# zju3dv/LoFTR

Hardware: AMD Instinct MI355X
Metric: image-pairs/sec @640x480 indoor-ds (higher is better)
Workload: dtype f32; 1 GPU; batch=8 640x480 synthetic grayscale pairs per GPU, indoor_ds dual-softmax (BASELINE configs[1]), full LoFTR.forward = ResNet-FPN backbone (HIP implicit-GEMM / patch convolutions incl. the 7x7 stem) + HIP matching path; weights=seeded random init (no checkpoint on the box), conf_matrix_materialised=True, match_type=dual_softmax, global_batch=8, parallelism=dp1 (pairs sharded; RCCL all-gather of match counts)

## Files before the change

loftr_amd/build.py:

```python
import os
import subprocess
import sys
from concurrent.futures import ThreadPoolExecutor

HERE = os.path.dirname(os.path.abspath(__file__))
CSRC = os.path.join(HERE, "csrc")
OBJ_DIR = os.path.join(CSRC, "build")
LIB_PATH = os.path.join(HERE, "libloftr_hip.so")
SOURCES = ["linear.hip", "coarse_plan.hip", "attention.hip", "transformer.hip", "coarse_match.hip", "fine.hip", "misc.hip",
           "sp_convert.hip", "conv.hip", "eval.hip", "input.hip", "comm.hip", "pose.hip", "train.hip", "train_bwd.hip", "encoder_fused.hip", "fine_fused.hip", "head_grads.hip", "encoder_bwd.hip", "fine_bwd.hip", "train_glue.hip", "bank.hip", "pose_gpu.hip", "window_head.hip", "window_head_first.hip", "geometry.hip", "geometry_gpu.hip", "absolute_pose.hip", "absolute_pose_gpu.hip", "atlas.hip", "atlas_gpu.hip", "triangulate.hip", "triangulate_gpu.hip", "model_lookup.hip", "model_lookup_gpu.hip", "bundle.hip", "bundle_gpu.hip", "register.hip", "register_gpu.hip"]
FLAGS = ["--offload-arch=gfx950", "-O3", "-std=c++17", "-fPIC", "-Wall", "-Wno-unused-parameter"]


def _hipcc():
    for c in (os.environ.get("HIPCC"), "/opt/rocm/bin/hipcc", "hipcc"):
        if c and (os.path.isabs(c) and os.path.exists(c) or not os.path.isabs(c)):
            return c
    raise RuntimeError("hipcc not found")


def _deps_mtime():
    paths = [os.path.join(CSRC, f) for f in os.listdir(CSRC) if f.endswith((".h", ".hip"))]
    paths.append(os.path.join(os.path.dirname(HERE), "include", "loftr_hip.h"))
    return max(os.path.getmtime(p) for p in paths)


def build(force=False, verbose=True, extra_flags=(), lib_path=None, obj_dir=None):
    global LIB_PATH, OBJ_DIR
    lib_default, obj_default = LIB_PATH, OBJ_DIR
    if lib_path:
        LIB_PATH, OBJ_DIR, force = lib_path, obj_dir or (OBJ_DIR + "_variant"), True
    try:
        return _build(force, verbose, tuple(extra_flags))
    finally:
        LIB_PATH, OBJ_DIR = lib_default, obj_default


def _build(force, verbose, extra_flags):
    if not force and os.path.exists(LIB_PATH) and os.path.getmtime(LIB_PATH) >= _deps_mtime():
        return LIB_PATH
    os.makedirs(OBJ_DIR, exist_ok=True)
    hipcc = _hipcc()

    def compile_one(src):
        obj = os.path.join(OBJ_DIR, src.replace(".hip", ".o"))
        cmd = [hipcc, *FLAGS, *extra_flags, "-c", os.path.join(CSRC, src), "-o", obj]
        r = subprocess.run(cmd, capture_output=True, text=True)
        if r.returncode != 0:
            raise RuntimeError(f"hipcc failed on {src}:\n{r.stderr}")
        if verbose and r.stderr.strip():
            sys.stderr.write(r.stderr)
        return obj

    with ThreadPoolExecutor(max_workers=min(8, len(SOURCES))) as ex:
        objs = list(ex.map(compile_one, SOURCES))
    vs = os.path.join(OBJ_DIR, "exports.map")
    with open(vs, "w") as fh:
        fh.write("{ global: loftr_*; local: *; };\n")
    r = subprocess.run([hipcc, "--offload-arch=gfx950", "-shared", "-fPIC", f"-Wl,--version-script={vs}", "-o", LIB_PATH, *objs, "-ldl"],
                       capture_output=True, text=True)
    if r.returncode != 0:
        raise RuntimeError(f"link failed:\n{r.stderr}")
    if verbose:
        print(f"built {LIB_PATH} ({os.path.getsize(LIB_PATH) / 1e6:.2f} MB)")
    return LIB_PATH


if __name__ == "__main__":
    if "--variant" in sys.argv:
        i = sys.argv.index("--variant")
        name = sys.argv[i + 1]
        build(extra_flags=[a for a in sys.argv[i + 2:] if a.startswith("-")],
              lib_path=os.path.join(HERE, f"libloftr_hip_{name}.so"), obj_dir=os.path.join(CSRC, "build", f"variant_{name}"))
    else:
        build(force="--force" in sys.argv)
```

loftr_amd/csrc/common.h:

```cpp
#pragma once
#include <hip/hip_runtime.h>
#include <stdint.h>
#include <stddef.h>
#include "../../include/loftr_hip.h"

typedef float f32x16 __attribute__((ext_vector_type(16)));
typedef float f32x4 __attribute__((ext_vector_type(4)));
typedef float f32x2 __attribute__((ext_vector_type(2)));

#define LOFTR_NEG_INF (-1e9f)

#define LOFTR_CHECK_ARG(cond) do { if (!(cond)) return LOFTR_ERR_BAD_ARG; } while (0)
#define LOFTR_CHECK_LAUNCH() do { if (hipGetLastError() != hipSuccess) return LOFTR_ERR_LAUNCH; } while (0)

#ifdef __HIP_DEVICE_COMPILE__
#define LOFTR_NO_PACKED_FP32 __attribute__((target("no-packed-fp32-ops")))
#else
#define LOFTR_NO_PACKED_FP32
#endif

__host__ __device__ static inline int ceil_div(int a, int b) { return (a + b - 1) / b; }
static inline size_t align_up(size_t x, size_t a) { return (x + a - 1) / a * a; }

enum LoftrTimedKernel {
  LOFTR_T_SCORE_STATS = 0,
  LOFTR_T_SCORE_CONF = 1,
  LOFTR_T_PROJ = 2,
  LOFTR_T_LINEAR = 3,
  LOFTR_T_LINEAR_LN = 4,
  LOFTR_T_KV = 5,
  LOFTR_T_ATTN_APPLY = 6,
  LOFTR_T_ATTN_SMALL = 7,
  LOFTR_T_GATHER = 8,
  LOFTR_T_OT_STORE = 9,
  LOFTR_T_CONV = 10,
  LOFTR_T_CONV3 = 11,
  LOFTR_T_CONV3W = 12,
  LOFTR_T_ENCODER_X = 13,
  LOFTR_T_FINE_PAIR = 14,
  LOFTR_T_COUNT = 15
};
enum LoftrDebugKey {
  LOFTR_DBG_ENCODER_SCHEDULE = 0,
  LOFTR_DBG_CONV_PERSIST_CAP,
  LOFTR_DBG_WGRAD_CHUNK,
  LOFTR_DBG_REDUCE_TALL,
  LOFTR_DBG_PCT_GRID,
  LOFTR_DBG_PCT_SKIP,
  LOFTR_DBG_PCT_QUOTA,
  LOFTR_DBG_CONV_DUO,
  LOFTR_DBG_CONV_PATCH,
  LOFTR_DBG_CONV_REM,
  LOFTR_DBG_COUNT
};
int loftr_debug_value(int key);
extern unsigned g_loftr_timing_mask;
extern int g_loftr_range_check;
void loftr_timing_mark(int id, hipStream_t st, bool end);
struct TimedLaunch {
  int id; hipStream_t st; bool on;
  TimedLaunch(int id_, hipStream_t st_) : id(id_), st(st_), on((g_loftr_timing_mask >> id_) & 1u) {
    if (on) loftr_timing_mark(id, st, false);
  }
  ~TimedLaunch() { if (on) loftr_timing_mark(id, st, true); }
};

constexpr int NUM_XCD = 8;
static inline unsigned xcd_grid(int tiles_m, int tiles_n) { return (unsigned)(NUM_XCD * ceil_div(tiles_m, NUM_XCD) * tiles_n); }
__device__ __forceinline__ bool xcd_tile(int tiles_m, int tiles_n, int& tile_m, int& tile_n) {
  const int id = blockIdx.x, xcd = id % NUM_XCD, slot = id / NUM_XCD;
  const int chunk = ceil_div(tiles_m, NUM_XCD);
  tile_n = slot % tiles_n;
  const int local = slot / tiles_n;
  tile_m = xcd * chunk + local;
  return local < chunk && tile_m < tiles_m;
}

struct WsAlloc {
  char* base; size_t cap; size_t off;
  WsAlloc(void* p, size_t bytes) : base((char*)p), cap(bytes), off(0) {}
  template <typename T> T* take(size_t n) {
    off = align_up(off, 256);
    T* r = (T*)(base + off);
    off += n * sizeof(T);
    return r;
  }
  bool ok() const { return off <= cap; }
};

__device__ __forceinline__ float wave_sum(float v) {
#pragma unroll
  for (int o = 32; o >= 1; o >>= 1) v += __shfl_xor(v, o, 64);
  return v;
}
__device__ __forceinline__ float wave_max(float v) {
#pragma unroll
  for (int o = 32; o >= 1; o >>= 1) v = fmaxf(v, __shfl_xor(v, o, 64));
  return v;
}
#define LOFTR_DPP(v_, ctrl_) __int_as_float(__builtin_amdgcn_update_dpp(0, __float_as_int(v_), ctrl_, 0xF, 0xF, true))
#define LOFTR_DPPI(v_, ctrl_) __builtin_amdgcn_update_dpp(0, v_, ctrl_, 0xF, 0xF, true)
__device__ __forceinline__ float half_sum(float v) {
  v += LOFTR_DPP(v, 0xB1);
  v += LOFTR_DPP(v, 0x4E);
  v += LOFTR_DPP(v, 0x141);
  v += LOFTR_DPP(v, 0x140);
  const auto r = __builtin_amdgcn_permlane16_swap(__float_as_int(v), __float_as_int(v), false, false);
  return __int_as_float(r[0]) + __int_as_float(r[1]);
}
__device__ __forceinline__ float half_max(float v) {
  v = fmaxf(v, LOFTR_DPP(v, 0xB1));
  v = fmaxf(v, LOFTR_DPP(v, 0x4E));
  v = fmaxf(v, LOFTR_DPP(v, 0x141));
  v = fmaxf(v, LOFTR_DPP(v, 0x140));
  const auto r = __builtin_amdgcn_permlane16_swap(__float_as_int(v), __float_as_int(v), false, false);
  return fmaxf(__int_as_float(r[0]), __int_as_float(r[1]));
}
__device__ __forceinline__ int half_min_i32(int v) {
  v = min(v, LOFTR_DPPI(v, 0xB1));
  v = min(v, LOFTR_DPPI(v, 0x4E));
  v = min(v, LOFTR_DPPI(v, 0x141));
  v = min(v, LOFTR_DPPI(v, 0x140));
  const auto r = __builtin_amdgcn_permlane16_swap(v, v, false, false);
  return min((int)r[0], (int)r[1]);
}
__device__ __forceinline__ void half_sum16(f32x16& v) {
#pragma unroll
  for (int r = 0; r < 16; ++r) v[r] += LOFTR_DPP(v[r], 0xB1);
#pragma unroll
  for (int r = 0; r < 16; ++r) v[r] += LOFTR_DPP(v[r], 0x4E);
#pragma unroll
  for (int r = 0; r < 16; ++r) v[r] += LOFTR_DPP(v[r], 0x141);
#pragma unroll
  for (int r = 0; r < 16; ++r) v[r] += LOFTR_DPP(v[r], 0x140);
#pragma unroll
  for (int r = 0; r < 16; ++r) {
    const auto q = __builtin_amdgcn_permlane16_swap(__float_as_int(v[r]), __float_as_int(v[r]), false, false);
    v[r] = __int_as_float(q[0]) + __int_as_float(q[1]);
  }
}
__device__ __forceinline__ void half_max16(f32x16& v) {
#pragma unroll
  for (int r = 0; r < 16; ++r) v[r] = fmaxf(v[r], LOFTR_DPP(v[r], 0xB1));
#pragma unroll
  for (int r = 0; r < 16; ++r) v[r] = fmaxf(v[r], LOFTR_DPP(v[r], 0x4E));
#pragma unroll
  for (int r = 0; r < 16; ++r) v[r] = fmaxf(v[r], LOFTR_DPP(v[r], 0x141));
#pragma unroll
  for (int r = 0; r < 16; ++r) v[r] = fmaxf(v[r], LOFTR_DPP(v[r], 0x140));
#pragma unroll
  for (int r = 0; r < 16; ++r) {
    const auto q = __builtin_amdgcn_permlane16_swap(__float_as_int(v[r]), __float_as_int(v[r]), false, false);
    v[r] = fmaxf(__int_as_float(q[0]), __int_as_float(q[1]));
  }
}
__device__ __forceinline__ float swap32(float v) {
  const auto r = __builtin_amdgcn_permlane32_swap(__float_as_int(v), __float_as_int(v), false, false);
  return __int_as_float((threadIdx.x & 32) ? r[0] : r[1]);
}
#define LOFTR_DPP_SWAP32(v_) swap32(v_)

__device__ __forceinline__ float elu1(float x) {
  return x > 0.f ? x + 1.f : __expf(x);
}
```

loftr_amd/csrc/conv.hip:

```cpp
#include "gemm.h"
#include "conv_prepared.h"
#include <stdlib.h>

namespace {

using CfgD = GemmCfg<256, 128, 4, 2, 3>;

struct ConvArgs {
  ASrc a;
  const sp_t* w; int K;
  const float* bias;
  const float* wscale;
  const float* x_inv;
  const sp_t* residual;
  sp_t* y_sp;
  float* y_f32;
  int M, Cout, Coutp;
  int act;
  const sp_t* up;
  int Hl, Wl;
  float sy, sx;
};

template <typename Cfg, bool FULL>
__device__ __forceinline__ void conv_epilogue(const ConvArgs& p, f32x16 (&acc)[Cfg::TM][Cfg::TN], int m0, int n0) {
  const EpiLane<Cfg> e;
  const sp_t* rs = p.residual ? p.residual + (long)m0 * p.Coutp + n0 : nullptr;
  sp_t* os = p.y_sp ? p.y_sp + (long)m0 * p.Coutp + n0 : nullptr;
  float* of = p.y_f32 ? p.y_f32 + (long)m0 * p.Cout + n0 : nullptr;
#pragma unroll
  for (int j = 0; j < Cfg::TN; ++j) {
    const int col = n0 + e.lcol + j * 32;
    const bool creal = col < p.Cout;
    const bool cpad = col < p.Coutp;
    const float b = (p.bias && creal) ? p.bias[col] : 0.f;
    const float wsc = (creal ? p.wscale[col] : 1.f) * (p.x_inv ? *p.x_inv : 1.f);
#pragma unroll
    for (int i = 0; i < Cfg::TM; ++i) {
      f32x16 v = acc[i][j] * wsc;
      if (rs) {
        uint32_t w[16];
#pragma unroll
        for (int r = 0; r < 16; ++r) {
          const int trow = e.lrow + e.rr(i, r);
          const bool ok = (FULL || m0 + trow < p.M) && cpad;
          w[r] = ok ? rs[(unsigned)(trow * p.Coutp + e.spcol + j * 32)] : 0u;
        }
#pragma unroll
        for (int r = 0; r < 16; ++r) v[r] += sp_value(w[r], e.odd);
      }
#pragma unroll
      for (int r = 0; r < 16; ++r) {
        float x = v[r] + b;
        if (p.act == 1) x = fmaxf(x, 0.f);
        if (p.act == 2) x = x > 0.f ? x : 0.01f * x;
        v[r] = creal ? x : 0.f;
      }
      if (of) {
#pragma unroll
        for (int r = 0; r < 16; ++r) {
          const int trow = e.lrow + e.rr(i, r);
          if ((FULL || m0 + trow < p.M) && creal) of[(unsigned)(trow * p.Cout + e.lcol + j * 32)] = v[r];
        }
      }
      if (os) {
        uint32_t w[16];
        sp_words16(v, e.odd, w);
#pragma unroll
        for (int r = 0; r < 16; ++r) {
          const int trow = e.lrow + e.rr(i, r);
          if ((FULL || m0 + trow < p.M) && cpad) os[(unsigned)(trow * p.Coutp + e.spcol + j * 32)] = w[r];
        }
      }
    }
  }
}

template <typename Cfg>
__device__ __forceinline__ void conv_epilogue_up(const ConvArgs& p, f32x16 (&acc)[Cfg::TM][Cfg::TN], int m0, int n0,
                                                 float* lds) {
  constexpr int LD = Cfg::BN + 4;
  static_assert(Cfg::BM * LD <= Cfg::LDS_FLOATS, "accumulator tile does not fit the operand ring");
  const EpiLane<Cfg> e;
  __syncthreads();
  const float xinv = p.x_inv ? *p.x_inv : 1.f;
#pragma unroll
  for (int j = 0; j < Cfg::TN; ++j) {
    const int col = n0 + e.lcol + j * 32;
    const float wsc = (col < p.Cout ? p.wscale[col] : 1.f) * xinv;
#pragma unroll
    for (int i = 0; i < Cfg::TM; ++i)
#pragma unroll
      for (int r = 0; r < 16; ++r) lds[(e.lrow + e.rr(i, r)) * LD + e.lcol + j * 32] = acc[i][j][r] * wsc;
  }
  __syncthreads();
  const int Wo = 2 * p.Wl, Ho = 2 * p.Hl;
  constexpr int OCTS = Cfg::BN / 8;
  for (int it = threadIdx.x; it < Cfg::BM * OCTS; it += Cfg::THREADS) {
    const int row = it / OCTS, oct = it - row * OCTS;
    const int pix = m0 + row, col0 = n0 + oct * 8;
    if (pix >= p.M || col0 >= p.Coutp) continue;
    const int t = pix / Wo, x = pix - t * Wo;
    const int bb = t / Ho, y = t - bb * Ho;
    const float fy = p.sy * (float)y, fx = p.sx * (float)x;
    const int y0 = (int)fy, x0 = (int)fx;
    const int dy = y0 < p.Hl - 1 ? p.Wl * p.Coutp : 0, dx = x0 < p.Wl - 1 ? p.Coutp : 0;
    const float ly = fy - (float)y0, lx = fx - (float)x0;
    const float hy = 1.f - ly, hx = 1.f - lx;
    const int off = sp_octet_off(col0 >> 3);
    const sp_t* s00 = p.up + (unsigned)(((bb * p.Hl + y0) * p.Wl + x0) * p.Coutp + off);
    const sp_t* src[4] = {s00, s00 + dx, s00 + dy, s00 + dy + dx};
    u32x4 hi[4], lo[4];
#pragma unroll
    for (int k = 0; k < 4; ++k) {
      hi[k] = *reinterpret_cast<const u32x4*>(src[k]);
      lo[k] = *reinterpret_cast<const u32x4*>(src[k] + 16);
    }
    float v[4][8], o[8];
#pragma unroll
    for (int k = 0; k < 4; ++k) sp_unpack8(hi[k], lo[k], v[k]);
    const f32x4 a0 = *reinterpret_cast<const f32x4*>(&lds[row * LD + oct * 8]);
    const f32x4 a1 = *reinterpret_cast<const f32x4*>(&lds[row * LD + oct * 8 + 4]);
#pragma unroll
    for (int c = 0; c < 8; ++c)
      o[c] = col0 + c < p.Cout
                 ? (c < 4 ? a0[c] : a1[c - 4]) + (hy * (hx * v[0][c] + lx * v[1][c]) + ly * (hx * v[2][c] + lx * v[3][c]))
                 : 0.f;
    u32x4 oh, ol;
    sp_pack8(o, oh, ol);
    sp_t* dst = p.y_sp + (unsigned)(pix * p.Coutp + off);
    *reinterpret_cast<u32x4*>(dst) = oh;
    *reinterpret_cast<u32x4*>(dst + 16) = ol;
  }
}

template <typename Cfg, bool UP>
__global__ __launch_bounds__(Cfg::THREADS, 2) void conv_kernel(ConvArgs p) {
  __shared__ __attribute__((aligned(16))) float lds[Cfg::LDS_FLOATS];
  int tm, tn;
  if (!xcd_tile(ceil_div(p.M, Cfg::BM), ceil_div(p.Coutp, Cfg::BN), tm, tn)) return;
  const int m0 = tm * Cfg::BM, n0 = tn * Cfg::BN;
  f32x16 acc[Cfg::TM][Cfg::TN];
  gemm_mainloop<Cfg, true>(p.a, p.w, p.K, p.M, p.Cout, p.K, m0, n0, lds, acc, p.Coutp);
  if constexpr (UP) conv_epilogue_up<Cfg>(p, acc, m0, n0, lds);
  else if (m0 + Cfg::BM <= p.M) conv_epilogue<Cfg, true>(p, acc, m0, n0);
  else conv_epilogue<Cfg, false>(p, acc, m0, n0);
}

namespace c3 {
constexpr int TY = 8, TX = 32, PW = TX + 2, PH = TY + 2, PROWS = PW * PH;
constexpr int PSLOTS = 43, PQ = 6;
constexpr int PATCH_BYTES = PSLOTS * 1024, BTILE_BYTES = 128 * 128;
constexpr int NB = 4;
constexpr int LDS_BYTES = 2 * PATCH_BYTES + NB * BTILE_BYTES + 1024;
// ... 462 lines not shown
}

template <int RT>
__global__ __launch_bounds__(256) void conv_rem_gather_kernel(const float* __restrict__ pbuf, long npix, int H, int W, int R, int c0, int Coutp,
                                                              const float* __restrict__ bias, const sp_t* __restrict__ residual, int act,
                                                              sp_t* __restrict__ y_sp) {
  const long pix = (long)blockIdx.x * 256 + threadIdx.x;
  if (pix >= npix) return;
  const int x = (int)(pix % W), y = (int)((pix / W) % H);
  float v[8];
#pragma unroll
  for (int c = 0; c < 8; ++c) v[c] = 0.f;
  const float* pp = pbuf + pix * (9 * R);
#pragma unroll
  for (int ky = 0; ky < 3; ++ky)
#pragma unroll
    for (int kx = 0; kx < 3; ++kx) {
      const int yy = y + ky - 1, xx = x + kx - 1;
      if ((unsigned)yy < (unsigned)H && (unsigned)xx < (unsigned)W) {
        const float* q = pp + ((long)(ky - 1) * W + (kx - 1)) * (9 * R) + (ky * 3 + kx) * R;
        if (RT == 4) {
          const f32x4 t = *reinterpret_cast<const f32x4*>(q);
          v[0] += t[0]; v[1] += t[1]; v[2] += t[2]; v[3] += t[3];
        } else {
#pragma unroll
          for (int c = 0; c < 7; ++c) if (c < R) v[c] += q[c];
        }
      }
    }
  sp_t* row = y_sp + pix * Coutp + c0;
  float rv[8];
#pragma unroll
  for (int c = 0; c < 8; ++c) rv[c] = 0.f;
  if (residual) {
    const sp_t* rr = residual + pix * Coutp + c0;
    const u32x4 hi = *reinterpret_cast<const u32x4*>(rr), lo = *reinterpret_cast<const u32x4*>(rr + 16);
    sp_unpack8(hi, lo, rv);
  }
  const float slope = act == 1 ? 0.f : act == 2 ? 0.01f : 1.f;
  float o[8];
#pragma unroll
  for (int c = 0; c < 8; ++c) {
    const float t = v[c] + ((bias && c < R) ? bias[c0 + c] : 0.f) + rv[c];
    o[c] = c < R ? fmaxf(t, slope * t) : 0.f;
  }
  u32x4 oh, ol;
  sp_pack8(o, oh, ol);
  const u32x4 z = {0u, 0u, 0u, 0u};
  u32x4* dst = reinterpret_cast<u32x4*>(row);
  dst[0] = oh; dst[1] = z; dst[2] = z; dst[3] = z; dst[4] = ol; dst[5] = z; dst[6] = z; dst[7] = z;
}


static int conv_prepare(const float* weight, const long* weight_strides, int Cin, int Cout, int KH, int KW,
                        const float* bn_weight, const float* bn_bias, const float* bn_mean, const float* bn_var, float bn_eps,
                        void* buf, size_t bytes, hipStream_t st) {
  LOFTR_CHECK_ARG(weight && weight_strides && buf && Cin > 0 && Cout > 0 && KH > 0 && KW > 0);
  LOFTR_CHECK_ARG((bn_weight == nullptr) == (bn_bias == nullptr) && (bn_weight == nullptr) == (bn_mean == nullptr) &&
                  (bn_weight == nullptr) == (bn_var == nullptr));
  ConvPrepared pr;
  if (!conv_prepared_layout(buf, bytes, Cin, Cout, KH, KW, pr)) return LOFTR_ERR_WORKSPACE;
  const int Cp = ceil32(Cin), K = KH * KW * Cp;
  (void)hipMemsetAsync(pr.zeros, 0, 256, st);
  hipLaunchKernelGGL(conv_rowscale_kernel, dim3(Cout), dim3(256), 0, st, weight, bn_weight, bn_bias, bn_mean, bn_var, bn_eps,
                     Cin, KH, KW, weight_strides[0], weight_strides[1], weight_strides[2], weight_strides[3], pr.bias, pr.wscale);
  hipLaunchKernelGGL(conv_prep_kernel, dim3(ceil_div(K / 32, 8), Cout), dim3(256), 0, st, weight, bn_weight, bn_bias,
                     bn_mean, bn_var, bn_eps, Cin, Cp, KH, KW, weight_strides[0], weight_strides[1], weight_strides[2],
                     weight_strides[3], pr.wsp, pr.wscale);
  LOFTR_CHECK_LAUNCH();
  return LOFTR_OK;
}

static int conv_rem_channels(int Cout, int KH, int KW, int stride) {
  return (KH == 3 && KW == 3 && stride == 1 && ceil32(Cout) == 224 && Cout - 192 >= 1 && Cout - 192 <= 7) ? Cout - 192 : 0;
}
extern "C" size_t loftr_conv_scratch_bytes(int B, int H, int W, int Cout, int KH, int KW, int stride) {
  const int R = conv_rem_channels(Cout, KH, KW, stride);
  return (R > 0 && B > 0 && H > 0 && W > 0) ? (size_t)B * H * W * 9 * R * 4 : 0;
}

static int conv_run(const uint32_t* x_sp, int B, int H, int W, int Cin, const void* prepared, size_t prepared_bytes, int Cout,
                    int KH, int KW, int stride, int pad, int act, const uint32_t* residual_sp, const uint32_t* up_sp,
                    uint32_t* y_sp, float* y_f32, void* stream, const float* x_inv = nullptr, void* scratch = nullptr, size_t scratch_bytes = 0) {
  LOFTR_CHECK_ARG(x_sp && prepared && (y_sp || y_f32) && B >= 0 && H > 0 && W > 0 && Cin > 0 && Cout > 0);
  const bool shared_gpu = (act & LOFTR_CONV_SHARED_GPU) != 0;
  act &= ~LOFTR_CONV_SHARED_GPU;
  LOFTR_CHECK_ARG(KH > 0 && KW > 0 && stride > 0 && pad >= 0 && act >= 0 && act <= 2);
  if (B == 0) return LOFTR_OK;
  hipStream_t st = (hipStream_t)stream;
  ConvGeom g;
  g.H = H; g.W = W; g.Cp = ceil32(Cin); g.KH = KH; g.KW = KW; g.stride = stride; g.pad = pad;
  g.Ho = (H + 2 * pad - KH) / stride + 1;
  g.Wo = (W + 2 * pad - KW) / stride + 1;
  if (g.Ho <= 0 || g.Wo <= 0 || H >= 32768 || W >= 32768) return LOFTR_ERR_UNSUPPORTED;
  if (up_sp && ((g.Ho & 1) || (g.Wo & 1) || KH != 1 || KW != 1 || stride != 1 || pad != 0 || !y_sp || y_f32 || residual_sp || act != 0))
    return LOFTR_ERR_UNSUPPORTED;
  const long M = (long)B * g.Ho * g.Wo;
  if (M * (long)ceil32(Cout) >= (1L << 31) || (long)B * H * W * g.Cp >= (1L << 31)) return LOFTR_ERR_UNSUPPORTED;
  const int K = KH * KW * g.Cp;
  ConvPrepared pr;
  if (!conv_prepared_layout(const_cast<void*>(prepared), prepared_bytes, Cin, Cout, KH, KW, pr)) return LOFTR_ERR_WORKSPACE;
  sp_t* wsp = pr.wsp;
  float* bias = pr.bias;
  sp_t* zeros = pr.zeros;
  g.zeros = zeros;
  ConvArgs p;
  p.a = asrc_conv(x_sp, g);
  p.w = wsp; p.K = K; p.bias = bias; p.wscale = pr.wscale; p.x_inv = x_inv; p.residual = residual_sp; p.y_sp = y_sp; p.y_f32 = y_f32;
  p.M = (int)M; p.Cout = Cout; p.Coutp = ceil32(Cout); p.act = act;
  p.up = up_sp; p.Hl = g.Ho / 2; p.Wl = g.Wo / 2;
  p.sy = g.Ho > 1 ? (float)(p.Hl - 1) / (float)(g.Ho - 1) : 0.f;
  p.sx = g.Wo > 1 ? (float)(p.Wl - 1) / (float)(g.Wo - 1) : 0.f;
  if (loftr_debug_value(LOFTR_DBG_CONV_PATCH) && KH == 3 && KW == 3 && stride == 1 && pad == 1 && !up_sp) {
    Conv3Args c;
    c.x = x_sp; c.B = B; c.H = H; c.W = W; c.Cp = g.Cp; c.Cin = Cin; c.w = wsp; c.K = K; c.bias = bias; c.wscale = pr.wscale; c.x_inv = x_inv; c.residual = residual_sp;
    c.y_sp = y_sp; c.y_f32 = y_f32; c.Cout = Cout; c.Coutp = ceil32(Cout); c.act = act; c.zeros = zeros;
    c.tiles_x = ceil_div(W, c3::TX); c.tiles_y = ceil_div(H, c3::TY); c.pbuf = nullptr;
    const bool duo = loftr_debug_value(LOFTR_DBG_CONV_DUO) != 0;
    const bool wide = duo && c.Coutp == 32 * 7;
    TimedLaunch tl(wide ? LOFTR_T_CONV3W : LOFTR_T_CONV3, st);
    if (duo && c.Coutp % 128 == 0) {
      using CF = c3d::Cfg<4, 2, 4>;
      c.tiles_y = ceil_div(H, CF::TY);
      hipLaunchKernelGGL((conv3x3_duo_kernel<CF>), dim3(xcd_grid(B * c.tiles_x * c.tiles_y, c.Coutp / 128)), dim3(256), 0, st, c);
    } else if (duo && c.Coutp == 192) {
      using CF = c3d::Cfg<6, 2, 4, 8, 2>;
      c.tiles_y = ceil_div(H, CF::TY);
      hipLaunchKernelGGL((conv3x3_duo_kernel<CF>), dim3(xcd_grid(B * c.tiles_x * c.tiles_y, 1)), dim3(512), 0, st, c);
    } else if (wide && conv_rem_channels(Cout, KH, KW, stride) > 0 && !y_f32 && loftr_debug_value(LOFTR_DBG_CONV_REM) &&
               scratch && scratch_bytes >= (size_t)B * H * W * 9 * conv_rem_channels(Cout, KH, KW, stride) * 4) {
      using CF = c3d::Cfg<6, 2, 4, 8, 2, true>;
      c.tiles_y = ceil_div(H, CF::TY);
      c.pbuf = reinterpret_cast<float*>(scratch);
      hipLaunchKernelGGL((conv3x3_duo_kernel<CF>), dim3(xcd_grid(B * c.tiles_x * c.tiles_y, 1)), dim3(512), 0, st, c);
      LOFTR_CHECK_LAUNCH();
      const long npix = (long)B * H * W;
      if (Cout - 192 == 4)
        hipLaunchKernelGGL(conv_rem_gather_kernel<4>, dim3((unsigned)((npix + 255) / 256)), dim3(256), 0, st, c.pbuf, npix, H, W, 4, 192, c.Coutp,
                           bias, residual_sp, act, y_sp);
      else
        hipLaunchKernelGGL(conv_rem_gather_kernel<0>, dim3((unsigned)((npix + 255) / 256)), dim3(256), 0, st, c.pbuf, npix, H, W, Cout - 192, 192, c.Coutp,
                           bias, residual_sp, act, y_sp);
    } else if (wide) {
      using CF = c3d::Cfg<7, 2, 4, 8, 2>;
      c.tiles_y = ceil_div(H, CF::TY);
      hipLaunchKernelGGL((conv3x3_duo_kernel<CF>), dim3(xcd_grid(B * c.tiles_x * c.tiles_y, 1)), dim3(512), 0, st, c);
    } else
      hipLaunchKernelGGL(conv3x3_kernel, dim3(shared_gpu ? xcd_grid(B * c.tiles_x * c.tiles_y, ceil_div(c.Coutp, 128))
                                                         : persistent_grid(xcd_grid(B * c.tiles_x * c.tiles_y, ceil_div(c.Coutp, 128)))),
                         dim3(512), 0, st, c);
    LOFTR_CHECK_LAUNCH();
    return LOFTR_OK;
  }
  {
    TimedLaunch tl(LOFTR_T_CONV, st);
    if (up_sp)
      hipLaunchKernelGGL((conv_kernel<CfgD, true>), dim3(xcd_grid(ceil_div(p.M, CfgD::BM), ceil_div(p.Coutp, CfgD::BN))),
                         dim3(CfgD::THREADS), 0, st, p);
    else
      hipLaunchKernelGGL((conv_kernel<CfgD, false>), dim3(xcd_grid(ceil_div(p.M, CfgD::BM), ceil_div(p.Coutp, CfgD::BN))),
                         dim3(CfgD::THREADS), 0, st, p);
  }
  LOFTR_CHECK_LAUNCH();
  return LOFTR_OK;
}

#ifdef LOFTR_CONV_PROBE
extern "C" int loftr_conv_probe_buffer(void* buf) {
  long long* b = (long long*)buf;
  return hipMemcpyToSymbol(HIP_SYMBOL(g_conv_probe), &b, sizeof(b)) == hipSuccess ? LOFTR_OK : LOFTR_ERR_LAUNCH;
}
#endif

extern "C" int loftr_conv_prepare(const float* weight, const long* weight_strides, int Cin, int Cout, int KH, int KW,
                                  const float* bn_weight, const float* bn_bias, const float* bn_mean, const float* bn_var,
                                  float bn_eps, void* prepared, size_t prepared_bytes, void* stream) {
  return conv_prepare(weight, weight_strides, Cin, Cout, KH, KW, bn_weight, bn_bias, bn_mean, bn_var, bn_eps, prepared,
                      prepared_bytes, (hipStream_t)stream);
}

extern "C" int loftr_conv_bn_act_prepared(const uint32_t* x_sp, int B, int H, int W, int Cin, const void* prepared,
                                          size_t prepared_bytes, int Cout, int KH, int KW, int stride, int pad, int act,
                                          const uint32_t* residual_sp, const uint32_t* low_sp, uint32_t* y_sp, float* y_f32,
                                          const float* x_inv_scale, void* stream) {
  return conv_run(x_sp, B, H, W, Cin, prepared, prepared_bytes, Cout, KH, KW, stride, pad, act, residual_sp, low_sp, y_sp, y_f32,
                  stream, x_inv_scale);
}

extern "C" int loftr_conv_bn_act_prepared_scratch(const uint32_t* x_sp, int B, int H, int W, int Cin, const void* prepared,
                                                  size_t prepared_bytes, int Cout, int KH, int KW, int stride, int pad, int act,
                                                  const uint32_t* residual_sp, const uint32_t* low_sp, uint32_t* y_sp, float* y_f32,
                                                  const float* x_inv_scale, void* scratch, size_t scratch_bytes, void* stream) {
  return conv_run(x_sp, B, H, W, Cin, prepared, prepared_bytes, Cout, KH, KW, stride, pad, act, residual_sp, low_sp, y_sp, y_f32,
                  stream, x_inv_scale, scratch, scratch_bytes);
}

extern "C" int loftr_conv_bn_act(const uint32_t* x_sp, int B, int H, int W, int Cin, const float* weight,
                                 const long* weight_strides, int Cout, int KH, int KW, int stride, int pad, const float* bn_weight, const float* bn_bias,
                                 const float* bn_mean, const float* bn_var, float bn_eps, int act,
                                 const uint32_t* residual_sp, uint32_t* y_sp, float* y_f32, void* ws, size_t ws_bytes,
                                 const float* x_inv_scale, void* stream) {
  LOFTR_CHECK_ARG(x_sp && (y_sp || y_f32) && B >= 0 && H > 0 && W > 0);
  if (B == 0) return LOFTR_OK;
  const int rc = conv_prepare(weight, weight_strides, Cin, Cout, KH, KW, bn_weight, bn_bias, bn_mean, bn_var, bn_eps, ws, ws_bytes,
                              (hipStream_t)stream);
  if (rc != LOFTR_OK) return rc;
  return conv_run(x_sp, B, H, W, Cin, ws, ws_bytes, Cout, KH, KW, stride, pad, act, residual_sp, nullptr, y_sp, y_f32, stream, x_inv_scale);
}

extern "C" int loftr_conv1x1_upsample_add(const uint32_t* x_sp, int B, int H, int W, int Cin, const float* weight,
                                          const long* weight_strides, int Cout, const uint32_t* low_sp, uint32_t* y_sp,
                                          void* ws, size_t ws_bytes, void* stream) {
  LOFTR_CHECK_ARG(x_sp && low_sp && y_sp && B >= 0 && H > 0 && W > 0);
  if (B == 0) return LOFTR_OK;
  const int rc = conv_prepare(weight, weight_strides, Cin, Cout, 1, 1, nullptr, nullptr, nullptr, nullptr, 0.f, ws, ws_bytes,
                              (hipStream_t)stream);
  if (rc != LOFTR_OK) return rc;
  return conv_run(x_sp, B, H, W, Cin, ws, ws_bytes, Cout, 1, 1, 1, 0, 0, nullptr, low_sp, y_sp, nullptr, stream);
}

extern "C" int loftr_stem_conv_bn_relu(const float* x, const long* x_strides, int B, int H, int W, const float* weight,
                                       const long* weight_strides, int C0, const float* bn_weight, const float* bn_bias,
                                       const float* bn_mean, const float* bn_var, float bn_eps, uint32_t* y_sp,
                                       void* stream) {
  LOFTR_CHECK_ARG(x && x_strides && weight && weight_strides && y_sp && B >= 0 && H > 0 && W > 0 && C0 > 0);
  LOFTR_CHECK_ARG((bn_weight == nullptr) == (bn_bias == nullptr) && (bn_weight == nullptr) == (bn_mean == nullptr) &&
                  (bn_weight == nullptr) == (bn_var == nullptr));
  if (C0 > 128) return LOFTR_ERR_UNSUPPORTED;
  if (B == 0) return LOFTR_OK;
  const int Ho = (H + 6 - 7) / 2 + 1, Wo = (W + 6 - 7) / 2 + 1;
  hipLaunchKernelGGL(stem_conv_kernel, dim3(ceil_div(Wo, STEM_TX), ceil_div(Ho, STEM_TY), B), dim3(256), 0,
                     (hipStream_t)stream, x, x_strides[0], x_strides[2], x_strides[3], H, W, weight, weight_strides[0],
                     weight_strides[2], weight_strides[3], bn_weight, bn_bias, bn_mean, bn_var, bn_eps, C0, Ho, Wo, y_sp);
  LOFTR_CHECK_LAUNCH();
  return LOFTR_OK;
}

extern "C" int loftr_upsample2x_add(const uint32_t* low_sp, const uint32_t* lateral_sp, uint32_t* out_sp, int B, int Hl,
                                    int Wl, int C, void* stream) {
  LOFTR_CHECK_ARG(low_sp && lateral_sp && out_sp && B >= 0 && Hl > 0 && Wl > 0 && C > 0);
  if (B == 0) return LOFTR_OK;
  const int Cp = ceil32(C);
  const long pixels = (long)B * 4 * Hl * Wl;
  if (pixels >= (1L << 31)) return LOFTR_ERR_UNSUPPORTED;
  const long nitems = pixels * (Cp / 8);
  if ((nitems + 255) / 256 >= (1L << 31)) return LOFTR_ERR_UNSUPPORTED;
  hipLaunchKernelGGL(upsample_add_kernel, dim3((unsigned)((nitems + 255) / 256)), dim3(256), 0, (hipStream_t)stream,
                     low_sp, lateral_sp, out_sp, Hl, Wl, Cp, nitems);
  LOFTR_CHECK_LAUNCH();
  return LOFTR_OK;
}

extern "C" int loftr_sp_from_f32(const float* src, uint32_t* dst_sp, long rows, int C, void* stream) {
  LOFTR_CHECK_ARG(src && dst_sp && rows >= 0 && C > 0);
  return launch_sp_convert1(src, C, dst_sp, rows, C, (hipStream_t)stream);
}

extern "C" int loftr_sp_from_f32_scaled(const float* src, uint32_t* dst_sp, long rows, int C, float* inv_scale_out, void* stream) {
  LOFTR_CHECK_ARG(src && dst_sp && inv_scale_out && rows >= 0 && C > 0);
  return launch_sp_convert1(src, C, dst_sp, rows, C, (hipStream_t)stream, inv_scale_out);
}

extern "C" int loftr_sp_to_f32(const uint32_t* src_sp, float* dst, long rows, int C, void* stream) {
  LOFTR_CHECK_ARG(src_sp && dst && rows >= 0 && C > 0);
  if (rows == 0) return LOFTR_OK;
  const int Cp = ceil32(C);
  hipLaunchKernelGGL(sp_to_f32_kernel, dim3((unsigned)rows), dim3(Cp > 256 ? 256 : Cp), 0, (hipStream_t)stream, src_sp,
                     dst, rows, C, Cp);
  LOFTR_CHECK_LAUNCH();
  return LOFTR_OK;
}
```

loftr_amd/csrc/misc.hip:

```cpp
#include "common.h"
#include <string.h>

namespace {
template <bool CL>
__global__ void pos_encode_flatten_kernel(loftr_fmap f, const float* __restrict__ pe,
                                          int pe_h, int pe_w, float* __restrict__ out, int C) {
  __shared__ float tile[32][33];
  const int H = f.H, W = f.W, HW = H * W;
  const int n = blockIdx.z, hw0 = blockIdx.x * 32, c0 = blockIdx.y * 32;
  const float* in = f.data + (long)n * f.sn;
  for (int k = threadIdx.y; k < 32; k += 8) {
    const int c = c0 + k, hw = hw0 + threadIdx.x;
    float v = 0.f;
    if (c < C && hw < HW) {
      const int y = hw / W, x = hw - y * W;
      v = pe[((long)c * pe_h + y) * pe_w + x];
      if (!CL) v += in[(long)c * f.sc + (long)y * f.sh + (long)x * f.sw];
    }
    tile[k][threadIdx.x] = v;
  }
  __syncthreads();
  for (int k = threadIdx.y; k < 32; k += 8) {
    const int hw = hw0 + k, c = c0 + threadIdx.x;
    if (hw < HW && c < C) {
      float v = tile[threadIdx.x][k];
      if (CL) { const int y = hw / W, x = hw - y * W; v += in[(long)y * f.sh + (long)x * f.sw + c]; }
      out[((long)n * HW + hw) * C + c] = v;
    }
  }
}
}

extern "C" int loftr_pos_encode_flatten(const loftr_fmap* feat, const float* pe, int pe_h, int pe_w, float* out,
                                        int N, int C, void* stream) {
  LOFTR_CHECK_ARG(feat && feat->data && pe && out && N >= 0 && C > 0 && feat->H > 0 && feat->W > 0 &&
                  feat->H <= pe_h && feat->W <= pe_w);
  if (N == 0) return LOFTR_OK;
  const dim3 grid(ceil_div(feat->H * feat->W, 32), ceil_div(C, 32), N), block(32, 8);
  if (feat->sc == 1)
    hipLaunchKernelGGL((pos_encode_flatten_kernel<true>), grid, block, 0, (hipStream_t)stream, *feat, pe, pe_h, pe_w, out, C);
  else
    hipLaunchKernelGGL((pos_encode_flatten_kernel<false>), grid, block, 0, (hipStream_t)stream, *feat, pe, pe_h, pe_w, out, C);
  LOFTR_CHECK_LAUNCH();
  return LOFTR_OK;
}

namespace {
struct DebugSwitch { const char* name; int def; int value; };
DebugSwitch g_debug[LOFTR_DBG_COUNT] = {{"encoder_schedule", 1, 1}, {"conv_persist_cap", 0, 0}, {"wgrad_chunk", 0, 0}, {"reduce_tall", 1, 1},
                                        {"pct_grid", 0, 0}, {"pct_skip", 0, 0}, {"pct_quota", 0, 0}, {"conv_duo", 1, 1}, {"conv_patch", 1, 1}, {"conv_rem", 1, 1}};
}
int loftr_debug_value(int key) { return (key >= 0 && key < LOFTR_DBG_COUNT) ? g_debug[key].value : 0; }
extern "C" int loftr_hip_debug_set(const char* key, int value) {
  LOFTR_CHECK_ARG(key != nullptr);
  for (auto& d : g_debug)
    if (strcmp(d.name, key) == 0) { d.value = value; return LOFTR_OK; }
  return LOFTR_ERR_BAD_ARG;
}
extern "C" int loftr_hip_debug_get(const char* key, int* value, int* default_value) {
  LOFTR_CHECK_ARG(key != nullptr && value != nullptr);
  for (auto& d : g_debug)
    if (strcmp(d.name, key) == 0) { *value = d.value; if (default_value) *default_value = d.def; return LOFTR_OK; }
  return LOFTR_ERR_BAD_ARG;
}

unsigned g_loftr_timing_mask = 0;
int g_loftr_range_check = 0;
extern "C" int loftr_hip_range_check_enable(int on) { g_loftr_range_check = on ? 1 : 0; return LOFTR_OK; }
namespace {
constexpr int T_POOL = 4096;
struct TimingSlot {
  hipEvent_t ev[T_POOL][2];
  int created, used;
  double total_ms; long long launches;
};
TimingSlot g_slots[LOFTR_T_COUNT];
const char* const T_NAMES[LOFTR_T_COUNT] = {"score_sweep_kernel<0>", "score_sweep_kernel<1>", "proj_kernel", "linear_kernel",
                                            "linear_ln_kernel", "proj_kv_kernel", "attn_apply_kernel",
                                            "attn_small_kernel", "gather_windows_kernel", "score_sweep_kernel<2>", "conv_kernel",
                                            "conv3x3_duo_kernel<Cfg<4,2,4,4,1>>", "conv3x3_duo_kernel<Cfg<7,2,4,8,2>>", "encoder_x_kernel", "fine_pair_kernel"};
void timing_drain(TimingSlot& s) {
  for (int i = 0; i < s.used; ++i) {
    float ms = 0.f;
    if (hipEventSynchronize(s.ev[i][1]) == hipSuccess && hipEventElapsedTime(&ms, s.ev[i][0], s.ev[i][1]) == hipSuccess) {
      s.total_ms += ms;
      s.launches += 1;
    }
  }
  s.used = 0;
}
}

void loftr_timing_mark(int id, hipStream_t st, bool end) {
  TimingSlot& s = g_slots[id];
  if (!end) {
    if (s.used >= T_POOL) return;
    if (s.used >= s.created) {
      if (hipEventCreate(&s.ev[s.created][0]) != hipSuccess || hipEventCreate(&s.ev[s.created][1]) != hipSuccess) return;
      s.created++;
    }
    (void)hipEventRecord(s.ev[s.used][0], st);
  } else {
    if (s.used >= s.created) return;
    (void)hipEventRecord(s.ev[s.used][1], st);
    s.used++;
  }
}

extern "C" int loftr_hip_timing_enable(unsigned mask) {
  g_loftr_timing_mask = mask & ((1u << LOFTR_T_COUNT) - 1u);
  return LOFTR_OK;
}

extern "C" int loftr_hip_timing_kernel_count(void) { return LOFTR_T_COUNT; }

extern "C" const char* loftr_hip_timing_kernel_name(int id) {
  return (id >= 0 && id < LOFTR_T_COUNT) ? T_NAMES[id] : "";
}

extern "C" int loftr_hip_timing_read(int id, double* total_ms, long long* launches, int reset) {
  LOFTR_CHECK_ARG(id >= 0 && id < LOFTR_T_COUNT && total_ms && launches);
  TimingSlot& s = g_slots[id];
  timing_drain(s);
  *total_ms = s.total_ms;
  *launches = s.launches;
  if (reset) { s.total_ms = 0.0; s.launches = 0; }
  return LOFTR_OK;
}

extern "C" int loftr_hip_abi_version(void) { return LOFTR_HIP_ABI_VERSION; }

extern "C" const char* loftr_hip_status_string(int status) {
  switch (status) {
    case LOFTR_OK: return "ok";
    case LOFTR_ERR_BAD_ARG: return "bad argument (null pointer or invalid shape)";
    case LOFTR_ERR_UNSUPPORTED: return "shape not supported by the gfx950 kernels";
    case LOFTR_ERR_WORKSPACE: return "workspace too small";
    case LOFTR_ERR_LAUNCH: return "HIP kernel launch failed";
    case LOFTR_ERR_NO_DEVICE: return "no gfx950 (MI355X) device";
    case LOFTR_ERR_COMM: return "RCCL unavailable or a communicator / collective call failed";
    case LOFTR_ERR_RANGE: return "an activation entering the split-fp16 GEMM chain is not below the fp16 maximum 65504 (or not finite)";
    default: return "unknown status";
  }
}

extern "C" int loftr_hip_device_check(void) {
  int dev = 0;
  if (hipGetDevice(&dev) != hipSuccess) return LOFTR_ERR_NO_DEVICE;
  hipDeviceProp_t prop;
  if (hipGetDeviceProperties(&prop, dev) != hipSuccess) return LOFTR_ERR_NO_DEVICE;
  return strncmp(prop.gcnArchName, "gfx950", 6) == 0 ? LOFTR_OK : LOFTR_ERR_NO_DEVICE;
}
```

Measured before the change: 452.7 image-pairs/s.

## Add persistent fused 1x1 conv + bilinear-upsample-add kernel for FPN top-down

Adds a dedicated persistent kernel for the FPN top-down lateral 1x1 conv that fuses the coarser-level bilinear upsample-and-add into the epilogue. It stages the upsample footprint into LDS with global_load_lds and double-buffers the K tiles. The next tile's loads are issued before the current epilogue runs, so loads and epilogue overlap. It is enabled by default through a new debug switch for Cp and Coutp up to 224, and otherwise falls back to the existing path. Risks include numerical differences in the interpolation order, and heavy LDS use per block may lower occupancy.

```diff
diff --git a/loftr_amd/build.py b/loftr_amd/build.py
--- a/loftr_amd/build.py
+++ b/loftr_amd/build.py
@@ -8,7 +8,7 @@
 OBJ_DIR = os.path.join(CSRC, "build")
 LIB_PATH = os.path.join(HERE, "libloftr_hip.so")
 SOURCES = ["linear.hip", "coarse_plan.hip", "attention.hip", "transformer.hip", "coarse_match.hip", "fine.hip", "misc.hip",
-           "sp_convert.hip", "conv.hip", "eval.hip", "input.hip", "comm.hip", "pose.hip", "train.hip", "train_bwd.hip", "encoder_fused.hip", "fine_fused.hip", "head_grads.hip", "encoder_bwd.hip", "fine_bwd.hip", "train_glue.hip", "bank.hip", "pose_gpu.hip", "window_head.hip", "window_head_first.hip", "geometry.hip", "geometry_gpu.hip", "absolute_pose.hip", "absolute_pose_gpu.hip", "atlas.hip", "atlas_gpu.hip", "triangulate.hip", "triangulate_gpu.hip", "model_lookup.hip", "model_lookup_gpu.hip", "bundle.hip", "bundle_gpu.hip", "register.hip", "register_gpu.hip"]
+           "sp_convert.hip", "conv.hip", "topdown.hip", "eval.hip", "input.hip", "comm.hip", "pose.hip", "train.hip", "train_bwd.hip", "encoder_fused.hip", "fine_fused.hip", "head_grads.hip", "encoder_bwd.hip", "fine_bwd.hip", "train_glue.hip", "bank.hip", "pose_gpu.hip", "window_head.hip", "window_head_first.hip", "geometry.hip", "geometry_gpu.hip", "absolute_pose.hip", "absolute_pose_gpu.hip", "atlas.hip", "atlas_gpu.hip", "triangulate.hip", "triangulate_gpu.hip", "model_lookup.hip", "model_lookup_gpu.hip", "bundle.hip", "bundle_gpu.hip", "register.hip", "register_gpu.hip"]
 FLAGS = ["--offload-arch=gfx950", "-O3", "-std=c++17", "-fPIC", "-Wall", "-Wno-unused-parameter"]
 
 
diff --git a/loftr_amd/csrc/common.h b/loftr_amd/csrc/common.h
--- a/loftr_amd/csrc/common.h
+++ b/loftr_amd/csrc/common.h
@@ -51,6 +51,7 @@
   LOFTR_DBG_CONV_DUO,
   LOFTR_DBG_CONV_PATCH,
   LOFTR_DBG_CONV_REM,
+  LOFTR_DBG_TOPDOWN_KERNEL,
   LOFTR_DBG_COUNT
 };
 int loftr_debug_value(int key);
diff --git a/loftr_amd/csrc/conv.hip b/loftr_amd/csrc/conv.hip
--- a/loftr_amd/csrc/conv.hip
+++ b/loftr_amd/csrc/conv.hip
@@ -1,5 +1,6 @@
 #include "gemm.h"
 #include "conv_prepared.h"
+#include "topdown.h"
 #include <stdlib.h>
 
 namespace {
@@ -768,6 +769,16 @@
     LOFTR_CHECK_LAUNCH();
     return LOFTR_OK;
   }
+  if (up_sp && loftr_debug_value(LOFTR_DBG_TOPDOWN_KERNEL) && topdown_applies(g.Cp, p.Coutp)) {
+    TopdownArgs t;
+    t.x = x_sp; t.w = wsp; t.wscale = pr.wscale; t.x_inv = x_inv; t.up = up_sp; t.y = y_sp;
+    t.B = B; t.Ho = g.Ho; t.Wo = g.Wo; t.Cp = g.Cp; t.Cout = Cout; t.Coutp = p.Coutp; t.Hl = p.Hl; t.Wl = p.Wl; t.sy = p.sy; t.sx = p.sx;
+    const unsigned nvirt = topdown_virtual_grid(t);
+    TimedLaunch tl(LOFTR_T_CONV, st);
+    topdown_launch(t, shared_gpu ? nvirt : persistent_grid(nvirt), st);
+    LOFTR_CHECK_LAUNCH();
+    return LOFTR_OK;
+  }
   {
     TimedLaunch tl(LOFTR_T_CONV, st);
     if (up_sp)
diff --git a/loftr_amd/csrc/misc.hip b/loftr_amd/csrc/misc.hip
--- a/loftr_amd/csrc/misc.hip
+++ b/loftr_amd/csrc/misc.hip
@@ -48,7 +48,8 @@
 namespace {
 struct DebugSwitch { const char* name; int def; int value; };
 DebugSwitch g_debug[LOFTR_DBG_COUNT] = {{"encoder_schedule", 1, 1}, {"conv_persist_cap", 0, 0}, {"wgrad_chunk", 0, 0}, {"reduce_tall", 1, 1},
-                                        {"pct_grid", 0, 0}, {"pct_skip", 0, 0}, {"pct_quota", 0, 0}, {"conv_duo", 1, 1}, {"conv_patch", 1, 1}, {"conv_rem", 1, 1}};
+                                        {"pct_grid", 0, 0}, {"pct_skip", 0, 0}, {"pct_quota", 0, 0}, {"conv_duo", 1, 1}, {"conv_patch", 1, 1}, {"conv_rem", 1, 1},
+                                        {"topdown_kernel", 1, 1}};
 }
 int loftr_debug_value(int key) { return (key >= 0 && key < LOFTR_DBG_COUNT) ? g_debug[key].value : 0; }
 extern "C" int loftr_hip_debug_set(const char* key, int value) {
diff --git a/loftr_amd/csrc/topdown.h b/loftr_amd/csrc/topdown.h
--- /dev/null
+++ b/loftr_amd/csrc/topdown.h
@@ -0,0 +1,18 @@
+#pragma once
+#include "gemm.h"
+
+struct TopdownArgs {
+  const sp_t* x;
+  const sp_t* w;
+  const float* wscale;
+  const float* x_inv;
+  const sp_t* up;
+  sp_t* y;
+  int B, Ho, Wo, Cp, Cout, Coutp, Hl, Wl;
+  float sy, sx;
+  int tiles_x, tiles_y, tiles_n, ncw;
+};
+
+bool topdown_applies(int Cp, int Coutp);
+unsigned topdown_virtual_grid(TopdownArgs& a);
+void topdown_launch(const TopdownArgs& a, unsigned grid, hipStream_t st);
diff --git a/loftr_amd/csrc/topdown.hip b/loftr_amd/csrc/topdown.hip
--- /dev/null
+++ b/loftr_amd/csrc/topdown.hip
@@ -0,0 +1,269 @@
+#include "topdown.h"
+
+namespace {
+
+namespace td {
+constexpr int TY = 4, TX = 32, FH = TY / 2 + 2, FW = TX / 2 + 2, FPIX = FH * FW;
+constexpr int A_BYTES = TY * TX * 128;
+}
+
+__device__ __forceinline__ float td_scale(float a, float s) {
+#pragma clang fp contract(off)
+  return a * s;
+}
+
+__device__ __forceinline__ float td_interp(float a, float pa, float pb, float qa, float qb, float vAa, float vAb, float vBa,
+                                           float vBb) {
+#pragma clang fp contract(off)
+  const float tA = __builtin_fmaf(pa, vAa, pb * vAb);
+  const float tB = __builtin_fmaf(pa, vBa, pb * vBb);
+  return a + __builtin_fmaf(qa, tA, qb * tB);
+}
+
+template <int NT>
+struct TdCfg {
+  static constexpr int TNW = (NT + 1) / 2;
+  static constexpr int NCW = NT * 32;
+  static constexpr int B_BYTES = NT * 4096, STAGE = td::A_BYTES + B_BYTES;
+  static constexpr int BGROUPS = NT * 4, BQ = TNW;
+  static constexpr int FSLOTS = td::FPIX * NT * 8 / 64, FQ = (FSLOTS + 7) / 8;
+  static constexpr int WS_OFF = 2 * STAGE + FSLOTS * 1024 + 1024;
+  static constexpr int LDS_BYTES = WS_OFF + 1024;
+  static_assert(td::FPIX * NT * 8 % 64 == 0, "footprint is a whole number of DMA instructions");
+  static_assert(LDS_BYTES <= 160 * 1024, "LDS");
+};
+
+template <int NT>
+__global__ __launch_bounds__(512) void topdown_kernel(TopdownArgs p) {
+  using namespace td;
+  using C = TdCfg<NT>;
+  constexpr int TNW = C::TNW, NCW = C::NCW, STAGE = C::STAGE, BQ = C::BQ, FQ = C::FQ;
+  typedef __attribute__((address_space(3))) void* lds_ptr_t;
+  typedef const __attribute__((address_space(1))) void* gbl_ptr_t;
+  __shared__ __attribute__((aligned(16))) char lds[C::LDS_BYTES];
+  char* const fp_base = lds + 2 * STAGE;
+  char* const scratch = fp_base + C::FSLOTS * 1024;
+  float* const wsl = reinterpret_cast<float*>(lds + C::WS_OFF);
+
+  const int tid = threadIdx.x, lane = tid & 63, wave = tid >> 6;
+  const int wm = wave & 3, wn = wave >> 2;
+  const int rsub = lane >> 3, slot = lane & 7;
+  const int g = lane >> 5, tx = lane & 31;
+  const bool odd = lane & 1;
+  const int nact = min(TNW, NT - wn * TNW);
+
+  const int tiles_m = p.B * p.tiles_y * p.tiles_x, tiles_n = p.tiles_n;
+  const int chunk_m = ceil_div(tiles_m, NUM_XCD), nvirt = NUM_XCD * chunk_m * tiles_n;
+  int vid = blockIdx.x;
+  int nb = 0, ny0 = 0, nx0 = 0, nn0 = 0;
+  bool have = false;
+#define TD_NEXT_TILE()                                                                                      \
+  {                                                                                                         \
+    have = false;                                                                                           \
+    for (; vid < nvirt; vid += gridDim.x) {                                                                 \
+      const int xcd__ = vid % NUM_XCD, slot__ = vid / NUM_XCD;                                              \
+      const int local__ = slot__ / tiles_n, tm__ = xcd__ * chunk_m + local__;                               \
+      if (local__ < chunk_m && tm__ < tiles_m) {                                                            \
+        nb = tm__ / (p.tiles_y * p.tiles_x);                                                                \
+        const int trem__ = tm__ - nb * (p.tiles_y * p.tiles_x);                                             \
+        ny0 = (trem__ / p.tiles_x) * TY; nx0 = (trem__ % p.tiles_x) * TX; nn0 = (slot__ % tiles_n) * p.ncw; \
+        have = true;                                                                                        \
+        break;                                                                                              \
+      }                                                                                                     \
+    }                                                                                                       \
+  }
+  TD_NEXT_TILE()
+  if (!have) return;
+
+  {
+    const float xinv = p.x_inv ? *p.x_inv : 1.f;
+    if (tid < 256) wsl[tid] = (tid < p.Cout ? p.wscale[tid] : 1.f) * xinv;
+    __syncthreads();
+  }
+
+  int aoff[2], boff[BQ], foff[FQ];
+#define TD_K_OFFSETS()                                                                                      \
+  {                                                                                                         \
+    _Pragma("unroll") for (int q = 0; q < 2; ++q) {                                                         \
+      const int r = (q * 8 + wave) * 8 + rsub;                      \
+      const int gy = min(ny0 + (r >> 5), p.Ho - 1), gx = min(nx0 + (r & 31), p.Wo - 1);                     \
+      aoff[q] = ((nb * p.Ho + gy) * p.Wo + gx) * p.Cp + ((slot ^ ((r >> 1) & 7)) << 2);                     \
+    }                                                                                                       \
+    _Pragma("unroll") for (int q = 0; q < BQ; ++q) {                                                        \
+      const int r = (q * 8 + wave) * 8 + rsub;                                                              \
+      boff[q] = min(nn0 + r, p.Cout - 1) * p.Cp + ((slot ^ ((r >> 1) & 7)) << 2);                           \
+    }                                                                                                       \
+  }
+#define TD_F_OFFSETS()                                                                                      \
+  {                                                                                                         \
+    const int fy0__ = (int)(p.sy * (float)ny0), fx0__ = (int)(p.sx * (float)nx0);                           \
+    _Pragma("unroll") for (int q = 0; q < FQ; ++q) {                                                        \
+      const int ci = (q * 8 + wave) * 64 + lane;                                                            \
+      const int fpix = ci / (NT * 8), c = ci - fpix * (NT * 8);                                             \
+      const int fr = min(fpix / FW, FH - 1), fc = fpix % FW;                                                \
+      const int gy = min(fy0__ + fr, p.Hl - 1), gx = min(fx0__ + fc, p.Wl - 1);                             \
+      foff[q] = ((nb * p.Hl + gy) * p.Wl + gx) * p.Coutp + nn0 + c * 4;                                     \
+    }                                                                                                       \
+  }
+#define TD_ISSUE_K(kt_, stage_)                                                                             \
+  {                                                                                                         \
+    char* s__ = lds + (stage_) * STAGE;                                                                     \
+    const int k0__ = (kt_) * 32;                                                                            \
+    _Pragma("unroll") for (int q = 0; q < 2; ++q)                                                           \
+      __builtin_amdgcn_global_load_lds((gbl_ptr_t)(p.x + (aoff[q] + k0__)), (lds_ptr_t)(s__ + (q * 8 + wave) * 1024), 16, 0, 0); \
+    _Pragma("unroll") for (int q = 0; q < BQ; ++q) {                                                        \
+      char* d__ = (q * 8 + wave < C::BGROUPS) ? s__ + A_BYTES + (q * 8 + wave) * 1024 : scratch;            \
+      __builtin_amdgcn_global_load_lds((gbl_ptr_t)(p.w + (boff[q] + k0__)), (lds_ptr_t)d__, 16, 0, 0);      \
+    }                                                                                                       \
+  }
+#define TD_ISSUE_F()                                                                                        \
+  {                                                                                                         \
+    _Pragma("unroll") for (int q = 0; q < FQ; ++q) {                                                        \
+      char* d__ = (q * 8 + wave < C::FSLOTS) ? fp_base + (q * 8 + wave) * 1024 : scratch;                   \
+      __builtin_amdgcn_global_load_lds((gbl_ptr_t)(p.up + foff[q]), (lds_ptr_t)d__, 16, 0, 0);              \
+    }                                                                                                       \
+  }
+
+  const int nk = p.Cp >> 5;
+  const int a_r = wm * 32 + tx;
+  const int b_r0 = wn * TNW * 32 + tx;
+  f32x16 acc[TNW];
+
+#define TD_LOOP(NJ_)                                                                                        \
+  for (int kt = 0; kt < nk; ++kt) {                                                                         \
+    if (kt == 0) LOFTR_WAITCNT_VM(FQ); else LOFTR_WAITCNT_VM(0);                                            \
+    __builtin_amdgcn_s_barrier();             \
+    if (kt + 1 < nk) TD_ISSUE_K(kt + 1, (kt + 1) & 1)                                                       \
+    const char* sA__ = lds + (kt & 1) * STAGE;                                                              \
+    const char* sB__ = sA__ + A_BYTES;                                                                      \
+    _Pragma("unroll") for (int ks = 0; ks < 2; ++ks) {                                                      \
+      h16x8 bh[(NJ_) > 0 ? (NJ_) : 1], bl[(NJ_) > 0 ? (NJ_) : 1];                                           \
+      const h16x8 ah = *reinterpret_cast<const h16x8*>(sA__ + lds_chunk_off(a_r, ks * 2 + g));              \
+      const h16x8 al = *reinterpret_cast<const h16x8*>(sA__ + lds_chunk_off(a_r, 4 + ks * 2 + g));          \
+      _Pragma("unroll") for (int j = 0; j < (NJ_); ++j) {                                                   \
+        bh[j] = *reinterpret_cast<const h16x8*>(sB__ + lds_chunk_off(b_r0 + j * 32, ks * 2 + g));           \
+        bl[j] = *reinterpret_cast<const h16x8*>(sB__ + lds_chunk_off(b_r0 + j * 32, 4 + ks * 2 + g));       \
+      }                                                                                                     \
+                                             \
+      _Pragma("unroll") for (int j = 0; j < (NJ_); ++j)                                                     \
+        acc[j] = __builtin_amdgcn_mfma_f32_32x32x16_f16(al, bh[j], acc[j], 0, 0, 0);                        \
+      _Pragma("unroll") for (int j = 0; j < (NJ_); ++j)                                                     \
+        acc[j] = __builtin_amdgcn_mfma_f32_32x32x16_f16(ah, bl[j], acc[j], 0, 0, 0);                        \
+      _Pragma("unroll") for (int j = 0; j < (NJ_); ++j)                                                     \
+        acc[j] = __builtin_amdgcn_mfma_f32_32x32x16_f16(ah, bh[j], acc[j], 0, 0, 0);                        \
+    }                                                                                                       \
+  }
+
+#define TD_EPILOGUE(NJ_)                                                                                    \
+  {                                                                                                         \
+    const uint32_t* fp__ = reinterpret_cast<const uint32_t*>(fp_base);                                      \
+    const int y = y0 + wm;                                                                                  \
+    const float fy = td_scale(p.sy, (float)y);        \
+    const int yl0 = (int)fy;                                                                                \
+    const float ly = fy - (float)yl0, hy = 1.f - ly;                                                        \
+    const int fyb = (int)(p.sy * (float)y0), fxb = (int)(p.sx * (float)x0);                                 \
+    const int r0 = min(yl0 - fyb, FH - 1), r1 = min(r0 + (yl0 < p.Hl - 1 ? 1 : 0), FH - 1);                 \
+    const bool swp = tx & 2;                  \
+    const float qa = swp ? hy : ly, qb = swp ? ly : hy;                                                     \
+    const int rA = swp ? r0 : r1, rB = swp ? r1 : r0;                                                       \
+    const int lidx = (wn * TNW) * 32 + (odd ? 16 : 0) + (tx >> 1);     \
+    float wsc[(NJ_) > 0 ? (NJ_) : 1];                                                                       \
+    bool creal[(NJ_) > 0 ? (NJ_) : 1];                                                                      \
+    _Pragma("unroll") for (int j = 0; j < (NJ_); ++j) {                                                     \
+      const int col = n0 + (wn * TNW + j) * 32 + tx;                                                        \
+      creal[j] = col < p.Cout;                             \
+      wsc[j] = wsl[col];                                                                                    \
+    }                                                                                                       \
+    _Pragma("unroll") for (int r = 0; r < 16; ++r) {                                                        \
+      const int x = x0 + (r & 3) + 8 * (r >> 2) + 4 * g;                                                    \
+      const float fx = td_scale(p.sx, (float)x);                                                            \
+      const int xl0 = (int)fx;                                                                              \
+      const float lx = fx - (float)xl0, hx = 1.f - lx;                                                      \
+      const int c0 = min(xl0 - fxb, FW - 1), c1 = min(c0 + (xl0 < p.Wl - 1 ? 1 : 0), FW - 1);               \
+      const float pa = swp ? lx : hx, pb = swp ? hx : lx;                                                   \
+      const int ca = swp ? c1 : c0, cb = swp ? c0 : c1;                                                     \
+      const int oAa = (rA * FW + ca) * NCW + lidx, oAb = (rA * FW + cb) * NCW + lidx;                       \
+      const int oBa = (rB * FW + ca) * NCW + lidx, oBb = (rB * FW + cb) * NCW + lidx;                       \
+      const bool ok = y < p.Ho && x < p.Wo;                                                                 \
+      sp_t* dst = p.y + (((b * p.Ho + min(y, p.Ho - 1)) * p.Wo + min(x, p.Wo - 1)) * p.Coutp + n0 + lidx);  \
+      uint32_t w[(NJ_) > 0 ? (NJ_) : 1];                                                                    \
+      _Pragma("unroll") for (int j = 0; j < (NJ_); ++j) {           \
+        const float vAa = sp_value(fp__[oAa + j * 32], odd), vAb = sp_value(fp__[oAb + j * 32], odd);       \
+        const float vBa = sp_value(fp__[oBa + j * 32], odd), vBb = sp_value(fp__[oBb + j * 32], odd);       \
+        const float a = td_scale(acc[j][r], wsc[j]);                                                        \
+        const float o = creal[j] ? td_interp(a, pa, pb, qa, qb, vAa, vAb, vBa, vBb) : 0.f;                  \
+        w[j] = sp_word(o, odd);                                                                             \
+      }                                                                                                     \
+      if (ok) {                                                                                             \
+        _Pragma("unroll") for (int j = 0; j < (NJ_); ++j) dst[j * 32] = w[j];                               \
+      }                                                                                                     \
+    }                                                                                                       \
+  }
+
+  TD_K_OFFSETS()
+  TD_F_OFFSETS()
+  TD_ISSUE_K(0, 0)
+  TD_ISSUE_F()
+  for (;;) {
+    const int b = nb, y0 = ny0, x0 = nx0, n0 = nn0;
+#pragma unroll
+    for (int j = 0; j < TNW; ++j)
+#pragma unroll
+      for (int r = 0; r < 16; ++r) acc[j][r] = 0.f;
+    if (nact == TNW) TD_LOOP(TNW)
+    else TD_LOOP(TNW - 1)
+    LOFTR_WAITCNT_VM(0);
+    __builtin_amdgcn_s_barrier();
+    vid += gridDim.x;
+    TD_NEXT_TILE()
+    if (have) {
+      TD_K_OFFSETS()
+      TD_ISSUE_K(0, 0)
+    }
+    if (nact == TNW) TD_EPILOGUE(TNW)
+    else TD_EPILOGUE(TNW - 1)
+    asm volatile("s_waitcnt lgkmcnt(0)" ::: "memory");
+    __builtin_amdgcn_s_barrier();
+    if (!have) break;
+    TD_F_OFFSETS()
+    TD_ISSUE_F()
+  }
+#undef TD_EPILOGUE
+#undef TD_LOOP
+#undef TD_ISSUE_F
+#undef TD_ISSUE_K
+#undef TD_F_OFFSETS
+#undef TD_K_OFFSETS
+#undef TD_NEXT_TILE
+}
+
+template <int NT>
+void td_launch(const TopdownArgs& a, unsigned grid, hipStream_t st) {
+  hipLaunchKernelGGL(topdown_kernel<NT>, dim3(grid), dim3(512), 0, st, a);
+}
+
+}
+
+bool topdown_applies(int Cp, int Coutp) {
+  return Cp >= 32 && Cp <= 224 && Cp % 32 == 0 && Coutp >= 32 && Coutp % 32 == 0 && Coutp <= 224;
+}
+
+unsigned topdown_virtual_grid(TopdownArgs& a) {
+  a.tiles_x = ceil_div(a.Wo, td::TX);
+  a.tiles_y = ceil_div(a.Ho, td::TY);
+  a.tiles_n = 1;
+  a.ncw = a.Coutp;
+  return xcd_grid(a.B * a.tiles_x * a.tiles_y, a.tiles_n);
+}
+
+void topdown_launch(const TopdownArgs& a, unsigned grid, hipStream_t st) {
+  switch (a.ncw / 32) {
+    case 1: td_launch<1>(a, grid, st); break;
+    case 2: td_launch<2>(a, grid, st); break;
+    case 3: td_launch<3>(a, grid, st); break;
+    case 4: td_launch<4>(a, grid, st); break;
+    case 5: td_launch<5>(a, grid, st); break;
+    case 6: td_launch<6>(a, grid, st); break;
+    default: td_launch<7>(a, grid, st); break;
+  }
+}
```

After: 449.0 image-pairs/s. No clear change (-0.8%).
